# Algomorph/LevelSetFusion-Python

Hardware: AMD Instinct MI355X
Metric: voxel-warp-updates/sec (higher is better)
Workload: dtype f32

## Files before the change

### levelsetfusion-python_amd/csrc/lsf_slavcheva.hip

```cpp
#include "lsf_device.h"

using namespace lsf;

#include "lsf_slavcheva_terms.h"

using namespace lsf::slav;

namespace {


template <int D, int SMOOTH, bool LEVELSET, int DATA, int ENERGY>
__device__ inline void voxel_gradient(const float* __restrict__ live, const float* __restrict__ canonical,
                                      const float* __restrict__ warp_prev, const Grid& g, const Params& p, int x,
                                      int y, int z, int i, float (&gv)[3], double (&en)[3]) {
    gv[0] = gv[1] = gv[2] = 0.0f;
    const float l = live[i], cn = canonical[i];
    if (fabsf(l) == 1.0f && fabsf(cn) == 1.0f) return;
    const bool interior = x > 0 && x < g.nx - 1 && y > 0 && y < g.ny - 1 && (D == 2 || (z > 0 && z < g.nz - 1));
    if (g.fast_ok && __all(interior)) {
        const NbhFast<D> n(live, warp_prev, g, x, y, z);
        band_voxel_gradient<D, SMOOTH, LEVELSET, DATA, ENERGY>(n, p, l, cn, gv, en);
    } else {
        const Nbh<D> n(live, warp_prev, g, x, y, z);
        band_voxel_gradient<D, SMOOTH, LEVELSET, DATA, ENERGY>(n, p, l, cn, gv, en);
// ... 295 lines not shown
}

__global__ __launch_bounds__(1024) void band_scan_kernel(int* __restrict__ sums_base, unsigned n, unsigned stride,
                                                         unsigned arrays, long long* totals,
                                                         const int* __restrict__ opposite) {
    if (blockIdx.x >= arrays) {
        reduce_opposite(opposite, n, totals);
        return;
    }
    __shared__ int wave_total[1024 / kWave];
    int* __restrict__ sums = sums_base + (size_t)blockIdx.x * stride;
    const unsigned t = threadIdx.x, lane = t & (kWave - 1), wave = t / kWave;
    int carry = 0;
    for (unsigned base = 0; base < n; base += 4096u) {
        const unsigned i = base + 4u * t;
        int v[4];
#pragma unroll
        for (int k = 0; k < 4; ++k) v[k] = i + k < n ? sums[i + k] : 0;
        const int mine = v[0] + v[1] + v[2] + v[3];
        int inclusive = mine;
#pragma unroll
        for (int d = 1; d < kWave; d <<= 1) {
            const int up = __shfl_up(inclusive, d, kWave);
            if ((int)lane >= d) inclusive += up;
        }
        if (lane == kWave - 1) wave_total[wave] = inclusive;
        __syncthreads();
        int before = 0, tile = 0;
#pragma unroll
        for (int w = 0; w < 1024 / kWave; ++w) {
            const int x = wave_total[w];
            before += w < (int)wave ? x : 0;
            tile += x;
        }
        int run = carry + before + inclusive - mine;
#pragma unroll
        for (int k = 0; k < 4; ++k) {
            if (i + k < n) sums[i + k] = run;
            run += v[k];
        }
        carry += tile;
        __syncthreads();
    }
    if (t == 0) totals[blockIdx.x] = carry;
}

constexpr unsigned kScanTile = 4096u;

__global__ __launch_bounds__(1024) void band_tile_totals_kernel(const int* __restrict__ sums_base, unsigned n,
                                                                unsigned stride, const int* __restrict__ opposite,
                                                                int* __restrict__ tile_out, unsigned tiles) {
    __shared__ int s_sum[1024 / kWave], s_first[1024 / kWave];
    const unsigned tile = blockIdx.x, a = blockIdx.y, t = threadIdx.x;
    const unsigned i = tile * kScanTile + 4u * t;
    int sum = 0, first = 0x7fffffff;
    if (a < 2u) {
        const int* __restrict__ sums = sums_base + (size_t)a * stride;
#pragma unroll
        for (unsigned k = 0; k < 4u; ++k) sum += i + k < n ? sums[i + k] : 0;
    } else {
#pragma unroll
        for (unsigned k = 0; k < 4u; ++k)
            if (i + k < n) {
                sum += opposite[2 * (i + k)];
                first = min(first, opposite[2 * (i + k) + 1]);
            }
    }
    for (int d = kWave / 2; d > 0; d >>= 1) {
        sum += __shfl_down(sum, d, kWave);
        first = min(first, __shfl_down(first, d, kWave));
    }
    if ((t & (kWave - 1)) == 0) {
        s_sum[t / kWave] = sum;
        s_first[t / kWave] = first;
    }
    __syncthreads();
    if (t == 0) {
        for (int k = 1; k < 1024 / kWave; ++k) {
            sum += s_sum[k];
            first = min(first, s_first[k]);
        }
        tile_out[(size_t)a * tiles + tile] = sum;
        if (a == 2u) tile_out[(size_t)3 * tiles + tile] = first;
    }
}

__global__ __launch_bounds__(1024) void band_scan_tiles_kernel(int* __restrict__ sums_base, unsigned n, unsigned stride,
                                                               const int* __restrict__ tile_out, unsigned tiles,
                                                               long long* __restrict__ totals, int zero_fifth) {
    const unsigned tile = blockIdx.x, a = blockIdx.y, t = threadIdx.x, lane = t & (kWave - 1), wave = t / kWave;
    if (a == 2u) {
        if (tile == 0u && t == 0u) {
            if (zero_fifth) totals[4] = 0;
            long long sum = 0;
            int first = 0x7fffffff;
            for (unsigned k = 0; k < tiles; ++k) {
                sum += tile_out[(size_t)2 * tiles + k];
                first = min(first, tile_out[(size_t)3 * tiles + k]);
            }
            totals[2] = sum;
            totals[3] = first == 0x7fffffff ? -1 : first;
        }
        return;
    }
    __shared__ int wave_total[1024 / kWave];
    int* __restrict__ sums = sums_base + (size_t)a * stride;
    int carry = 0;
    for (unsigned k = 0; k < tile; ++k) carry += tile_out[(size_t)a * tiles + k];
    const unsigned i = tile * kScanTile + 4u * t;
    int v[4];
#pragma unroll
    for (int k = 0; k < 4; ++k) v[k] = i + k < n ? sums[i + k] : 0;
    const int mine = v[0] + v[1] + v[2] + v[3];
    int inclusive = mine;
#pragma unroll
    for (int d = 1; d < kWave; d <<= 1) {
        const int up = __shfl_up(inclusive, d, kWave);
        if ((int)lane >= d) inclusive += up;
    }
    if (lane == kWave - 1) wave_total[wave] = inclusive;
    __syncthreads();
    int before = 0, whole = 0;
#pragma unroll
    for (int w = 0; w < 1024 / kWave; ++w) {
        const int x = wave_total[w];
        before += w < (int)wave ? x : 0;
        whole += x;
    }
    int run = carry + before + inclusive - mine;
#pragma unroll
    for (int k = 0; k < 4; ++k) {
        if (i + k < n) sums[i + k] = run;
        run += v[k];
    }
    if (tile == tiles - 1u && t == 0u) totals[a] = (long long)carry + whole;
}

typedef float vf4 __attribute__((ext_vector_type(4)));

__global__ __launch_bounds__(kBlock) void state_prepare_kernel(const float* __restrict__ live,
                                                               const float* __restrict__ canonical,
                                                               vf4* __restrict__ a, vf4* __restrict__ b, unsigned n,
                                                               Grid g, int dims, int* __restrict__ sums_interior,
                                                               int* __restrict__ sums_boundary,
                                                               unsigned long long* __restrict__ masks,
                                                               int* __restrict__ opposite, int* __restrict__ nonempty) {
    __shared__ int part[4][16];
    const int t = threadIdx.x, wave = t / kWave, lane = t % kWave;
#pragma unroll
    for (int j = 0; j < 4; ++j) {
        const unsigned v = blockIdx.x * kBandChunk + j * kBlock + t;
        bool in_band = false, interior = false, opposed = false;
        if (v < n) {
            const float l = live[v], cn = canonical[v];
            in_band = !(fabsf(l) == 1.0f && fabsf(cn) == 1.0f);
            opposed = !in_band && l != cn;
            vf4 o;
            o.x = l; o.y = 0.0f; o.z = 0.0f; o.w = 0.0f;
            if (a) a[v] = o;
            if (b) b[v] = o;
            const unsigned zy = fast_div(v, g.div_nx);
            const int x = (int)(v - zy * (unsigned)g.nx);
            const int z = (int)fast_div(zy, g.div_ny);
            const int y = (int)zy - z * g.ny;
            interior = x > 0 && x < g.nx - 1 && y > 0 && y < g.ny - 1 && (dims == 2 || (z > 0 && z < g.nz - 1));
        }
        const unsigned long long mi = __ballot(in_band && interior), mb = __ballot(in_band && !interior);
        const unsigned long long mo = __ballot(opposed);
        if (lane == 0) {
            part[0][j * 4 + wave] = __popcll(mi);
            part[1][j * 4 + wave] = __popcll(mb);
            part[2][j * 4 + wave] = __popcll(mo);
            part[3][j * 4 + wave] = mo ? (int)(blockIdx.x * kBandChunk + j * kBlock + wave * kWave) + __ffsll((long long)mo) - 1
                                       : 0x7fffffff;
            masks[((size_t)blockIdx.x * 16 + j * 4 + wave) * 2 + 0] = mi;
            masks[((size_t)blockIdx.x * 16 + j * 4 + wave) * 2 + 1] = mb;
        }
    }
    __syncthreads();
    if (t < 2) {
        int sum = 0;
        for (int k = 0; k < 16; ++k) sum += part[t][k];
        (t == 0 ? sums_interior : sums_boundary)[blockIdx.x] = sum;
    } else if (t == 2) {
        int sum = 0, first = 0x7fffffff;
        for (int k = 0; k < 16; ++k) {
            sum += part[2][k];
            first = min(first, part[3][k]);
        }
        opposite[2 * blockIdx.x] = sum;
        opposite[2 * blockIdx.x + 1] = first;
    } else if (t == 3) {
        int any = 0;
        for (int k = 0; k < 16; ++k) any |= part[0][k] | part[1][k];
        nonempty[blockIdx.x] = any != 0;
    }
}

constexpr int kPrepareChunksPerBlock = 4;
__device__ inline unsigned long long row16_or(unsigned nibble, int lane) {
    const int pos = lane & 15;
    unsigned lo = pos < 8 ? nibble << (4 * pos) : 0u, hi = pos < 8 ? 0u : nibble << (4 * (pos - 8));
#pragma unroll
    for (int d = 1; d < 16; d <<= 1) {
        lo |= (unsigned)__shfl_xor((int)lo, d, kWave);
        hi |= (unsigned)__shfl_xor((int)hi, d, kWave);
    }
    return ((unsigned long long)hi << 32) | lo;
}

__global__ __launch_bounds__(kBlock) void state_prepare4_kernel(const vf4* __restrict__ live4,
                                                                const vf4* __restrict__ canonical4,
                                                                vf4* __restrict__ a, vf4* __restrict__ b, unsigned n,
                                                                unsigned chunks, Grid g, int dims,
                                                                int* __restrict__ sums_interior,
                                                                int* __restrict__ sums_boundary,
                                                                unsigned long long* __restrict__ masks,
                                                                int* __restrict__ opposite, int* __restrict__ nonempty) {
    __shared__ int part[kPrepareChunksPerBlock][4][16];
    const int t = threadIdx.x, wave = t / kWave, lane = t % kWave;
    const unsigned chunk0 = blockIdx.x * kPrepareChunksPerBlock;
    vf4 l[kPrepareChunksPerBlock], c[kPrepareChunksPerBlock];
#pragma unroll
    for (int k = 0; k < kPrepareChunksPerBlock; ++k) {
        const unsigned v = (chunk0 + k) * kBandChunk + 4u * t;
        const vf4 one = {1.0f, 1.0f, 1.0f, 1.0f};
        l[k] = v < n ? live4[v / 4] : one;
        c[k] = v < n ? canonical4[v / 4] : one;
    }
#pragma unroll
    for (int k = 0; k < kPrepareChunksPerBlock; ++k) {
        const unsigned chunk = chunk0 + k, v = chunk * kBandChunk + 4u * t;
        unsigned ni = 0u, nb = 0u, no = 0u;
        if (v < n) {
            const unsigned zy = fast_div(v, g.div_nx);
            const int x0 = (int)(v - zy * (unsigned)g.nx);
            const int z = (int)fast_div(zy, g.div_ny);
            const int y = (int)zy - z * g.ny;
            const bool row_inside = y > 0 && y < g.ny - 1 && (dims == 2 || (z > 0 && z < g.nz - 1));
            const float lv[4] = {l[k].x, l[k].y, l[k].z, l[k].w}, cv[4] = {c[k].x, c[k].y, c[k].z, c[k].w};
#pragma unroll
            for (int j = 0; j < 4; ++j) {
                const bool in_band = !(fabsf(lv[j]) == 1.0f && fabsf(cv[j]) == 1.0f);
                const bool interior = row_inside && x0 + j > 0 && x0 + j < g.nx - 1;
                ni |= (in_band && interior ? 1u : 0u) << j;
                nb |= (in_band && !interior ? 1u : 0u) << j;
                no |= (!in_band && lv[j] != cv[j] ? 1u : 0u) << j;
                vf4 o;
                o.x = lv[j]; o.y = 0.0f; o.z = 0.0f; o.w = 0.0f;
                if (a) a[v + j] = o;
                if (b) b[v + j] = o;
            }
        }
        const unsigned long long mi = row16_or(ni, lane), mb = row16_or(nb, lane), mo = row16_or(no, lane);
        if ((lane & 15) == 0 && chunk < chunks) {
            const int word = wave * 4 + lane / 16;
            part[k][0][word] = __popcll(mi);
            part[k][1][word] = __popcll(mb);
            part[k][2][word] = __popcll(mo);
            part[k][3][word] = mo ? (int)(chunk * kBandChunk + word * kWave) + __ffsll((long long)mo) - 1 : 0x7fffffff;
            masks[((size_t)chunk * 16 + word) * 2 + 0] = mi;
            masks[((size_t)chunk * 16 + word) * 2 + 1] = mb;
        }
    }
    __syncthreads();
    if (t < 4 * kPrepareChunksPerBlock) {
        const int k = t / 4, what = t % 4;
        const unsigned chunk = chunk0 + k;
        if (chunk < chunks) {
            if (what < 2) {
                int sum = 0;
                for (int w = 0; w < 16; ++w) sum += part[k][what][w];
                (what == 0 ? sums_interior : sums_boundary)[chunk] = sum;
            } else if (what == 2) {
                int sum = 0, first = 0x7fffffff;
                for (int w = 0; w < 16; ++w) {
                    sum += part[k][2][w];
                    first = min(first, part[k][3][w]);
                }
                opposite[2 * chunk] = sum;
                opposite[2 * chunk + 1] = first;
            } else {
                int any = 0;
                for (int w = 0; w < 16; ++w) any |= part[k][0][w] | part[k][1][w];
                nonempty[chunk] = any != 0;
            }
        }
    }
}

__device__ inline bool chunk_is_needed(unsigned c, unsigned chunks, long long row, long long slice, int dims, int reach,
                                       const int* __restrict__ nonempty) {
    const int lane = threadIdx.x % kWave;
    const long long c0 = (long long)c * kBandChunk;
    const int span = 2 * reach + 1, zs = dims == 3 ? span : 1;
    bool hit = false;
    for (int k = lane; k < zs * span; k += kWave) {
        const int dy = k % span - reach, dz = dims == 3 ? k / span - reach : 0;
        const long long lo = c0 + dz * slice + dy * row - reach, hi = c0 + (long long)kBandChunk - 1 + dz * slice + dy * row + reach;
        long long first = lo >= 0 ? lo / kBandChunk : -((-lo + kBandChunk - 1) / kBandChunk);
        long long last = hi >= 0 ? hi / kBandChunk : -((-hi + kBandChunk - 1) / kBandChunk);
        first = first < 0 ? 0 : first;
        last = last >= (long long)chunks ? (long long)chunks - 1 : last;
        for (long long cand = first; cand <= last; ++cand) hit |= nonempty[cand] != 0;
    }
    return __any(hit);
}

constexpr int kPackChunks = 1;
static_assert(kPackChunks <= kBlock / kWave, "a wave per chunk of the block forms the verdicts");
__global__ __launch_bounds__(kBlock) void state_pack_needed_kernel(const float* __restrict__ live, vf4* __restrict__ a,
                                                                   vf4* __restrict__ b, unsigned n, unsigned chunks,
                                                                   int* __restrict__ needed, int want, int reach,
                                                                   long long row, long long slice, int dims,
                                                                   const int* __restrict__ nonempty) {
    const int t = threadIdx.x;
    __shared__ int s_verdict[kPackChunks];
    if (reach > 0) {
        const int k = t / kWave;
        const unsigned c = blockIdx.x * kPackChunks + k;
        if (k < kPackChunks && c < chunks) {
            const int any = chunk_is_needed(c, chunks, row, slice, dims, reach, nonempty) ? 1 : 0;
            if (t % kWave == 0) {
                needed[c] = any;
                s_verdict[k] = any;
            }
        }
        __syncthreads();
    }
    int verdict[kPackChunks];
#pragma unroll
    for (int k = 0; k < kPackChunks; ++k) {
        const unsigned c = blockIdx.x * kPackChunks + k;
        verdict[k] = c < chunks ? (reach > 0 ? s_verdict[k] : needed[c]) : -1;
    }
#pragma unroll
    for (int k = 0; k < kPackChunks; ++k) {
        if (verdict[k] != want) continue;
        const unsigned c = blockIdx.x * kPackChunks + k;
#pragma unroll
        for (int j = 0; j < 4; ++j) {
            const unsigned v = c * kBandChunk + j * kBlock + t;
            if (v < n) {
                vf4 o;
                o.x = live[v]; o.y = 0.0f; o.z = 0.0f; o.w = 0.0f;
                if (a) a[v] = o;
                if (b) b[v] = o;
            }
        }
    }
}



__global__ __launch_bounds__(kBlock) void band_fill_from_masks_kernel(const unsigned long long* __restrict__ masks,
                                                                      const int* __restrict__ block_sums, int which,
                                                                      int* __restrict__ list, unsigned chunks) {
    const int lane = threadIdx.x % kWave;
    const unsigned chunk = blockIdx.x * (kBlock / kWave) + threadIdx.x / kWave;
    if (chunk >= chunks) return;
    const unsigned long long mine = lane < 16 ? masks[((size_t)chunk * 16 + lane) * 2 + which] : 0ull;
    if (__ballot(mine != 0ull) == 0ull) return;
    int at = block_sums[chunk];
#pragma unroll
    for (int w = 0; w < 16; ++w) {
        const unsigned lo = (unsigned)__shfl((int)(unsigned)mine, w, kWave);
        const unsigned hi = (unsigned)__shfl((int)(unsigned)(mine >> 32), w, kWave);
        const unsigned long long m = ((unsigned long long)hi << 32) | lo;
        if ((m >> lane) & 1ull)
            list[at + __popcll(m & ((1ull << lane) - 1ull))] = (int)(chunk * kBandChunk + w * kWave + lane);
        at += __popcll(m);
    }
}

}

static inline bool band_subset_ok(int32_t subset) {
    return subset == LSF_BAND_ALL || subset == LSF_BAND_INTERIOR || subset == LSF_BAND_BOUNDARY;
}

extern "C" int lsf_slavcheva_gradient(const float* live, const float* canonical, const float* warp_prev_planar,
                                      float* g_out_planar, const lsf_grid* grid, const lsf_slavcheva_params* params,
                                      const lsf_gate* gate, lsf_iteration_record* record, const int32_t* band_list,
                                      int64_t band_count, void* stream) {
    if (int e = check_grid(grid)) return e;
    if (!live || !canonical || !warp_prev_planar || !params || !record || !g_out_planar ||
        g_out_planar == warp_prev_planar || (band_list && (band_count < 0 || band_count > 0x7fffffffll)))
        return LSF_ERR_BAD_ARGUMENT;
    Grid g = make_grid(grid);
    Tiling t = make_tiling(g);
    if (t.total == 0) return 0;
    LaunchArgs a{band_list ? band_list_blocks((unsigned)band_count) : launch_blocks(t.total), as_stream(stream), live,
                 canonical, warp_prev_planar, g_out_planar, g, make_params(params), gate_or_open(gate), record, band_list,
                 (unsigned)band_count};
    if (grid->dims == 2) pick_terms<2>(params, a);
    else pick_terms<3>(params, a);
    return launch_status();
}

extern "C" int lsf_slavcheva_update_rewarp(const float* live, const float* canonical, float* g_planar,
                                           float* warp_out_planar, float* live_out, const lsf_grid* grid,
                                           const lsf_slavcheva_params* params, const lsf_gate* gate,
                                           lsf_iteration_record* record, const int32_t* band_list, int64_t band_count,
                                           void* stream) {
    (void)canonical;
    if (int e = check_grid(grid)) return e;
    if (!live || !g_planar || !warp_out_planar || !live_out || live_out == live || !params || !record ||
        (band_list && (band_count < 0 || band_count > 0x7fffffffll)))
        return LSF_ERR_BAD_ARGUMENT;
    Grid g = make_grid(grid);
    Tiling t = make_tiling(g);
    if (t.total == 0) return 0;
    Params p = make_params(params);
    lsf_gate gt = gate_or_open(gate);
    const unsigned blocks = band_list ? band_list_blocks((unsigned)band_count) : launch_blocks(t.total);
    if (grid->dims == 2)
        hipLaunchKernelGGL(slavcheva_update_rewarp_kernel<2>, dim3(blocks), dim3(kBlock), 0, as_stream(stream), live,
                           g_planar, warp_out_planar, live_out, g, p, gt, record, band_list, (unsigned)band_count);
    else
        hipLaunchKernelGGL(slavcheva_update_rewarp_kernel<3>, dim3(blocks), dim3(kBlock), 0, as_stream(stream), live,
                           g_planar, warp_out_planar, live_out, g, p, gt, record, band_list, (unsigned)band_count);
    return launch_status();
}

template <int D, int NT>
static void launch_filter_update(bool fma, unsigned blocks, hipStream_t s, const float* in, const float* mask,
                                 const float* live, float* g_out, float* warp_out, float* live_out, const Grid& g,
                                 const Params& p, const double* taps_host, int axis, const lsf_gate& gt,
                                 lsf_iteration_record* record, const int* list, unsigned count) {
    TapsN<NT> taps;
    for (int j = 0; j < NT; ++j) taps.k[j] = taps_host[j];
    if (fma)
        hipLaunchKernelGGL((slavcheva_filter_update_rewarp_kernel<D, NT, true>), dim3(blocks), dim3(kBlock), 0, s, in, mask,
                           live, g_out, warp_out, live_out, g, p, taps, axis, gt, record, list, count);
    else
        hipLaunchKernelGGL((slavcheva_filter_update_rewarp_kernel<D, NT, false>), dim3(blocks), dim3(kBlock), 0, s, in, mask,
                           live, g_out, warp_out, live_out, g, p, taps, axis, gt, record, list, count);
}

extern "C" int lsf_slavcheva_filter_update_rewarp(const float* in_planar, const float* zero_mask_source,
                                                  const float* live, float* g_out_planar, float* warp_out_planar,
                                                  float* live_out, const lsf_grid* grid,
                                                  const lsf_slavcheva_params* params, int32_t axis,
                                                  const double* taps_host, int32_t n_taps, const lsf_gate* gate,
                                                  lsf_iteration_record* record, const int32_t* band_list,
                                                  int64_t band_count, void* stream) {
    if (int e = check_grid(grid)) return e;
    if (!in_planar || !zero_mask_source || !live || !g_out_planar || !warp_out_planar || !live_out ||
        live_out == live || g_out_planar == in_planar || !params || !record || !taps_host || !band_list ||
        band_count < 0 || band_count > 0x7fffffffll || axis < 0 || axis >= grid->dims)
        return LSF_ERR_BAD_ARGUMENT;
    if (n_taps != 3 && n_taps != 5 && n_taps != 7 && n_taps != 9) return LSF_ERR_KERNEL_TOO_LONG;
    Grid g = make_grid(grid);
    if (g.z_end == g.z_begin) return 0;
    const Params p = make_params(params);
    const lsf_gate gt = gate_or_open(gate);
    const unsigned blocks = band_list_blocks((unsigned)band_count);
    hipStream_t s = as_stream(stream);
    bool fma = true;
    for (int j = 0; j < n_taps; ++j) fma = fma && (double)(float)taps_host[j] == taps_host[j];
    const int* list = band_list;
    const unsigned count = (unsigned)band_count;
#define LSF_FUR(D, NT) launch_filter_update<D, NT>(fma, blocks, s, in_planar, zero_mask_source, live, g_out_planar, \
                                                 warp_out_planar, live_out, g, p, taps_host, axis, gt, record, list, count)
    if (grid->dims == 2) {
        switch (n_taps) { case 3: LSF_FUR(2, 3); break; case 5: LSF_FUR(2, 5); break; case 7: LSF_FUR(2, 7); break; default: LSF_FUR(2, 9); break; }
    } else {
        switch (n_taps) { case 3: LSF_FUR(3, 3); break; case 5: LSF_FUR(3, 5); break; case 7: LSF_FUR(3, 7); break; default: LSF_FUR(3, 9); break; }
    }
#undef LSF_FUR
    return launch_status();
}

static inline bool band_range(const lsf_grid* grid, unsigned& first, unsigned& n, unsigned& chunks) {
    const long long slice = (long long)grid->ny * grid->nx;
    first = (unsigned)(slice * grid->z_begin);
    n = (unsigned)(slice * (grid->z_end - grid->z_begin));
    chunks = (n + kBandChunk - 1) / kBandChunk;
    return n > 0;
}

extern "C" int64_t lsf_band_scratch_elements(const lsf_grid* grid) {
    if (check_grid(grid)) return 0;
    unsigned first, n, chunks;
    band_range(grid, first, n, chunks);
    return (int64_t)chunks + 1;
}

extern "C" int lsf_band_count(const float* live, const float* canonical, const lsf_grid* grid, int32_t subset,
                              int32_t* scratch, int64_t* count_out, void* stream) {
    if (int e = check_grid(grid)) return e;
    if (!live || !canonical || !scratch || !count_out || !band_subset_ok(subset)) return LSF_ERR_BAD_ARGUMENT;
    unsigned first, n, chunks;
    band_range(grid, first, n, chunks);
    hipStream_t s = as_stream(stream);
    if (chunks > 0)
        hipLaunchKernelGGL(band_list_kernel<false>, dim3(chunks), dim3(kBlock), 0, s, live, canonical, first, n,
                           make_grid(grid), grid->dims, subset, scratch, (int*)nullptr);
    hipLaunchKernelGGL(band_scan_kernel, dim3(1), dim3(1024), 0, s, scratch, chunks, 0u, 1u, (long long*)count_out,
                       (const int*)nullptr);
    return launch_status();
}

static inline unsigned long long* prepare_masks(int32_t* scratch, unsigned chunks) {
    return reinterpret_cast<unsigned long long*>(scratch + 2 * (size_t)(chunks + 1) + (2 * (chunks + 1)) % 2);
}

static inline int* prepare_opposite(int32_t* scratch, unsigned chunks) {
    return reinterpret_cast<int*>(prepare_masks(scratch, chunks) + (size_t)chunks * 32);
}

static inline int* prepare_nonempty(int32_t* scratch, unsigned chunks) { return prepare_opposite(scratch, chunks) + 2 * (size_t)chunks; }
static inline int* prepare_needed(int32_t* scratch, unsigned chunks) { return prepare_nonempty(scratch, chunks) + chunks; }
static inline unsigned prepare_scan_tiles(unsigned chunks) { return (chunks + kScanTile - 1u) / kScanTile; }
static inline int* prepare_tile_totals(int32_t* scratch, unsigned chunks) { return prepare_needed(scratch, chunks) + chunks; }

extern "C" int64_t lsf_state_prepare_scratch_elements(const lsf_grid* grid) {
    if (check_grid(grid, true)) return 0;
    unsigned first, n, chunks;
    band_range(grid, first, n, chunks);
    return 2 * (int64_t)(chunks + 1) + 64 * (int64_t)chunks + 2 + 2 * (int64_t)chunks + 2 * (int64_t)chunks +
           4 * ((int64_t)prepare_scan_tiles(chunks) + 1);
}

extern "C" int lsf_band_list_fill_prepared(const lsf_grid* grid, int32_t subset, const int32_t* scratch, int32_t* list,
                                           void* stream) {
    if (int e = check_grid(grid, true)) return e;
    if (!scratch || !list || (subset != LSF_BAND_INTERIOR && subset != LSF_BAND_BOUNDARY) || grid->z_begin != 0 ||
        grid->z_end != grid->nz)
        return LSF_ERR_BAD_ARGUMENT;
    unsigned first, n, chunks;
    if (!band_range(grid, first, n, chunks)) return 0;
    const int which = subset == LSF_BAND_INTERIOR ? 0 : 1;
    hipLaunchKernelGGL(band_fill_from_masks_kernel, dim3((chunks + kBlock / kWave - 1) / (kBlock / kWave)), dim3(kBlock),
                       0, as_stream(stream), prepare_masks(const_cast<int32_t*>(scratch), chunks),
                       scratch + which * (size_t)(chunks + 1), which, list, chunks);
    return launch_status();
}

namespace {
constexpr int kBoxGroup = kBlock;

__device__ inline unsigned long long box_mask_of(const unsigned long long* __restrict__ masks, unsigned box, int nbx,
                                                 int nby, int nx, int ny, bool all) {
    const int bx = (int)(box % (unsigned)nbx), by = (int)((box / (unsigned)nbx) % (unsigned)nby);
    const int bz = (int)(box / ((unsigned)nbx * (unsigned)nby));
    unsigned long long m = 0ull;
#pragma unroll
    for (int k = 0; k < 4; ++k)
#pragma unroll
        for (int j = 0; j < 4; ++j) {
            const unsigned v = (unsigned)(((4 * bz + k) * ny + 4 * by + j) * nx + 4 * bx);
            const unsigned long long word = masks[2 * (size_t)(v >> 6)] | (all ? masks[2 * (size_t)(v >> 6) + 1] : 0ull);
            m |= ((word >> (v & 63u)) & 0xFull) << (4 * (k * 4 + j));
        }
    return m;
}

template <bool FILL>
__global__ __launch_bounds__(kBlock) void band_boxes_kernel(const unsigned long long* __restrict__ masks, unsigned n_boxes,
                                                            int nbx, int nby, int nx, int ny, bool all,
                                                            int* __restrict__ group_sums, lsf_band_box* __restrict__ boxes) {
    __shared__ int wave_count[kBlock / kWave];
    const unsigned box = blockIdx.x * kBoxGroup + threadIdx.x;
    const int lane = threadIdx.x % kWave, wave = threadIdx.x / kWave;
    const unsigned long long m = box < n_boxes ? box_mask_of(masks, box, nbx, nby, nx, ny, all) : 0ull;
    const unsigned long long any = __ballot(m != 0ull);
    if (lane == 0) wave_count[wave] = __popcll(any);
    __syncthreads();
    if (!FILL) {
        if (threadIdx.x == 0) {
            int sum = 0;
            for (int k = 0; k < kBlock / kWave; ++k) sum += wave_count[k];
            group_sums[blockIdx.x] = sum;
        }
        return;
    }
    if (m == 0ull) return;
    int at = group_sums[blockIdx.x];
    for (int k = 0; k < wave; ++k) at += wave_count[k];
    at += __popcll(any & ((1ull << lane) - 1ull));
    const int bx = (int)(box % (unsigned)nbx), by = (int)((box / (unsigned)nbx) % (unsigned)nby);
    const int bz = (int)(box / ((unsigned)nbx * (unsigned)nby));
    lsf_band_box b;
    b.origin = ((4 * bz) * ny + 4 * by) * nx + 4 * bx;
    b.reserved = 0;
    b.mask = m;
    boxes[at] = b;
}

inline bool boxes_ok(const lsf_grid* g) {
    return g->dims == 3 && g->nx % 4 == 0 && g->ny % 4 == 0 && g->nz % 4 == 0 && g->z_begin == 0 && g->z_end == g->nz &&
           (long long)g->nx * g->ny * g->nz <= 0x0fffffffll;
}
}

extern "C" int64_t lsf_band_boxes_scratch_elements(const lsf_grid* grid) {
    if (check_grid(grid) || !boxes_ok(grid)) return 0;
    const long long n_boxes = (long long)grid->nx * grid->ny * grid->nz / 64;
    return (n_boxes + kBoxGroup - 1) / kBoxGroup + 1;
}

extern "C" int lsf_band_boxes_count(const lsf_grid* grid, int32_t subset, const int32_t* prepare_scratch,
                                    int32_t* box_scratch, int64_t* count_out, void* stream) {
    if (int e = check_grid(grid)) return e;
    if (!boxes_ok(grid)) return LSF_ERR_BAD_DIMS;
    if (!prepare_scratch || !box_scratch || !count_out || (subset != LSF_BAND_INTERIOR && subset != LSF_BAND_ALL))
        return LSF_ERR_BAD_ARGUMENT;
    unsigned first, n, chunks;
    band_range(grid, first, n, chunks);
    const unsigned n_boxes = n / 64, groups = (n_boxes + kBoxGroup - 1) / kBoxGroup;
    hipStream_t s = as_stream(stream);
    hipLaunchKernelGGL(band_boxes_kernel<false>, dim3(groups), dim3(kBlock), 0, s,
                       prepare_masks(const_cast<int32_t*>(prepare_scratch), chunks), n_boxes, grid->nx / 4, grid->ny / 4,
                       grid->nx, grid->ny, subset == LSF_BAND_ALL, box_scratch, (lsf_band_box*)nullptr);
    hipLaunchKernelGGL(band_scan_kernel, dim3(1), dim3(1024), 0, s, box_scratch, groups, 0u, 1u, (long long*)count_out,
                       (const int*)nullptr);
    return launch_status();
}

extern "C" int lsf_band_boxes_fill(const lsf_grid* grid, int32_t subset, const int32_t* prepare_scratch,
                                   const int32_t* box_scratch, lsf_band_box* boxes, void* stream) {
    if (int e = check_grid(grid)) return e;
    if (!boxes_ok(grid)) return LSF_ERR_BAD_DIMS;
    if (!prepare_scratch || !box_scratch || !boxes || (subset != LSF_BAND_INTERIOR && subset != LSF_BAND_ALL))
        return LSF_ERR_BAD_ARGUMENT;
    unsigned first, n, chunks;
    band_range(grid, first, n, chunks);
    const unsigned n_boxes = n / 64, groups = (n_boxes + kBoxGroup - 1) / kBoxGroup;
    hipLaunchKernelGGL(band_boxes_kernel<true>, dim3(groups), dim3(kBlock), 0, as_stream(stream),
                       prepare_masks(const_cast<int32_t*>(prepare_scratch), chunks), n_boxes, grid->nx / 4, grid->ny / 4,
                       grid->nx, grid->ny, subset == LSF_BAND_ALL, const_cast<int32_t*>(box_scratch), boxes);
    return launch_status();
}

extern "C" int lsf_state_prepare(const float* live, const float* canonical, float* state_a, float* state_b,
                                 const lsf_grid* grid, int32_t* scratch, int64_t* counts_out, void* stream) {
    return state_prepare_launch(live, canonical, state_a, state_b, grid, scratch, counts_out, false, stream);
}

int lsf::state_prepare_launch(const float* live, const float* canonical, float* state_a, float* state_b, const lsf_grid* grid,
                              int32_t* scratch, int64_t* counts_out, bool zero_fifth, void* stream) {
    if (int e = check_grid(grid, true)) return e;
    if (!live || !canonical || (!state_a && state_b) || !scratch || !counts_out) return LSF_ERR_BAD_ARGUMENT;
    if (grid->z_begin != 0 || grid->z_end != grid->nz) return LSF_ERR_BAD_ARGUMENT;
    unsigned first, n, chunks;
    band_range(grid, first, n, chunks);
    hipStream_t s = as_stream(stream);
    int* sums_interior = scratch;
    int* sums_boundary = scratch + (chunks + 1);
    const bool wide = grid->nx % 4 == 0 && ((uintptr_t)live | (uintptr_t)canonical) % 16 == 0;
    if (wide)
        hipLaunchKernelGGL(state_prepare4_kernel, dim3((chunks + kPrepareChunksPerBlock - 1) / kPrepareChunksPerBlock),
                           dim3(kBlock), 0, s, reinterpret_cast<const vf4*>(live), reinterpret_cast<const vf4*>(canonical),
                           reinterpret_cast<vf4*>(state_a), reinterpret_cast<vf4*>(state_b), n, chunks, make_grid(grid),
                           grid->dims, sums_interior, sums_boundary, prepare_masks(scratch, chunks),
                           prepare_opposite(scratch, chunks), prepare_nonempty(scratch, chunks));
    else
        hipLaunchKernelGGL(state_prepare_kernel, dim3(chunks), dim3(kBlock), 0, s, live, canonical,
                           reinterpret_cast<vf4*>(state_a), reinterpret_cast<vf4*>(state_b), n, make_grid(grid), grid->dims,
                           sums_interior, sums_boundary, prepare_masks(scratch, chunks), prepare_opposite(scratch, chunks),
                           prepare_nonempty(scratch, chunks));
    const unsigned tiles = prepare_scan_tiles(chunks) > 0u ? prepare_scan_tiles(chunks) : 1u;
    hipLaunchKernelGGL(band_tile_totals_kernel, dim3(tiles, 3), dim3(1024), 0, s, scratch, chunks, chunks + 1,
                       (const int*)prepare_opposite(scratch, chunks), prepare_tile_totals(scratch, chunks), tiles);
    hipLaunchKernelGGL(band_scan_tiles_kernel, dim3(tiles, 3), dim3(1024), 0, s, scratch, chunks, chunks + 1,
                       (const int*)prepare_tile_totals(scratch, chunks), tiles, (long long*)counts_out, zero_fifth ? 1 : 0);
    return launch_status();
}

extern "C" int lsf_state_pack_needed(const float* live, float* state_a, float* state_b, const lsf_grid* grid,
                                     int32_t* scratch, int32_t reach, int32_t invert, void* stream) {
    if (int e = check_grid(grid, true)) return e;
    if (!live || (!state_a && !state_b) || !scratch || reach < 1 || reach > 8) return LSF_ERR_BAD_ARGUMENT;
    if (grid->z_begin != 0 || grid->z_end != grid->nz) return LSF_ERR_BAD_ARGUMENT;
    unsigned first, n, chunks;
    band_range(grid, first, n, chunks);
    hipLaunchKernelGGL(state_pack_needed_kernel, dim3((chunks + kPackChunks - 1) / kPackChunks), dim3(kBlock), 0,
                       as_stream(stream), live, reinterpret_cast<vf4*>(state_a), reinterpret_cast<vf4*>(state_b), n, chunks,
                       prepare_needed(scratch, chunks), invert ? 0 : 1, invert ? 0 : (int)reach, (long long)grid->nx,
                       (long long)grid->nx * grid->ny, grid->dims, (const int*)prepare_nonempty(scratch, chunks));
    return launch_status();
}

extern "C" int lsf_band_list_fill(const float* live, const float* canonical, const lsf_grid* grid, int32_t subset,
                                  const int32_t* scratch, int32_t* list, void* stream) {
    if (int e = check_grid(grid)) return e;
    if (!live || !canonical || !scratch || !list || !band_subset_ok(subset)) return LSF_ERR_BAD_ARGUMENT;
    unsigned first, n, chunks;
    if (!band_range(grid, first, n, chunks)) return 0;
    hipLaunchKernelGGL(band_list_kernel<true>, dim3(chunks), dim3(kBlock), 0, as_stream(stream), live, canonical, first, n,
                       make_grid(grid), grid->dims, subset, const_cast<int32_t*>(scratch), list);
    return launch_status();
}
```

### levelsetfusion-python_amd/device.py

```python
import ctypes

import numpy as np
import torch

from . import _lib
from ._lib import Gate, Grid, HierParams, SlavchevaParams, check, lib
from .device_core import *
from .device_core import _PINNED, _gate_ref, _ptr, _record_ptr
from .device_fields import *
from .device_terms import term_gradient

def hier_iteration(packed, canonical, warp, g_prev, g_out, grid, params, gate, records, index):
    n = n_voxels(grid)
    n_packed = params.packed_nz * grid.ny * grid.nx if params.packed_nz > 0 else n
    check(lib.lsf_hier_iteration(_ptr(packed, 4 * n_packed, "packed live"), _ptr(canonical, n, "canonical"),
                                 _ptr(warp, n * grid.dims, "warp"),
                                 _ptr(g_prev, n * grid.dims, "g_prev", allow_none=True),
                                 _ptr(g_out, n * grid.dims, "g_out", allow_none=True), ctypes.byref(grid),
                                 ctypes.byref(params), _gate_ref(gate), _record_ptr(records, index), stream_ptr()),
          "lsf_hier_iteration")


def hier_update(g, warp, grid, rate, gate, records, index):
    n = n_voxels(grid) * grid.dims
    check(lib.lsf_hier_update(_ptr(g, n, "g"), _ptr(warp, n, "warp", allow_none=True), ctypes.byref(grid), float(rate),
                              _gate_ref(gate), _record_ptr(records, index), stream_ptr()), "lsf_hier_update")


class BandList:

    def __init__(self, indices, count, subset=_lib.BAND_ALL):
        self.indices, self.count, self.subset = indices, int(count), int(subset)
        self.pointer = ctypes.c_void_p(indices.data_ptr() if indices is not None else 0)

    @classmethod
    def none(cls):
        return cls(None, 0)


def buffer_addressing_ok(grid, bytes_per_voxel=16):
    if bytes_per_voxel != 16:
        return bytes_per_voxel * n_voxels(grid) < 0xffffffff
    return n_voxels(grid) < 0x7fffffff and 16 * (2 * grid.nx * grid.ny + 2 * grid.nx + 3) < 0x7fffffff


def band_lists(live, canonical, grid=None, split=True, bytes_per_voxel=16):
    grid = grid or make_grid(live.shape)
    n = n_voxels(grid)
    subsets = (_lib.BAND_INTERIOR, _lib.BAND_BOUNDARY) if split and buffer_addressing_ok(grid, bytes_per_voxel) \
        else (_lib.BAND_ALL,)
    n_scratch = int(lib.lsf_band_scratch_elements(ctypes.byref(grid)))
    scratch = torch.empty((len(subsets), n_scratch), dtype=torch.int32, device=live.device)
    totals = torch.zeros(len(subsets), dtype=torch.int64, device=live.device)
    p_live, p_canon = _ptr(live, n, "live"), _ptr(canonical, n, "canonical")
    for k, subset in enumerate(subsets):
        check(lib.lsf_band_count(p_live, p_canon, ctypes.byref(grid), subset, ctypes.c_void_p(scratch[k].data_ptr()),
                                 ctypes.c_void_p(totals[k:].data_ptr()), stream_ptr()), "lsf_band_count")
    counts = [int(c) for c in totals.cpu()]
    lists = []
    for k, (subset, count) in enumerate(zip(subsets, counts)):
        if count == 0 and not (k == len(subsets) - 1 and not lists):
            continue
        indices = torch.empty(max(count, 1), dtype=torch.int32, device=live.device)
        if count:
            check(lib.lsf_band_list_fill(p_live, p_canon, ctypes.byref(grid), subset,
                                         ctypes.c_void_p(scratch[k].data_ptr()), ctypes.c_void_p(indices.data_ptr()),
                                         stream_ptr()), "lsf_band_list_fill")
        lists.append(BandList(indices, count, subset))
    return lists


def band_list(live, canonical, grid=None, subset=_lib.BAND_ALL):
    grid = grid or make_grid(live.shape)
    n = n_voxels(grid)
    scratch = torch.empty(int(lib.lsf_band_scratch_elements(ctypes.byref(grid))), dtype=torch.int32,
                          device=live.device)
    total = torch.zeros(1, dtype=torch.int64, device=live.device)
    p_live, p_canon = _ptr(live, n, "live"), _ptr(canonical, n, "canonical")
    check(lib.lsf_band_count(p_live, p_canon, ctypes.byref(grid), int(subset), ctypes.c_void_p(scratch.data_ptr()),
                             ctypes.c_void_p(total.data_ptr()), stream_ptr()), "lsf_band_count")
    count = int(total.item())
    indices = torch.empty(max(count, 1), dtype=torch.int32, device=live.device)
    if count:
        check(lib.lsf_band_list_fill(p_live, p_canon, ctypes.byref(grid), int(subset),
                                     ctypes.c_void_p(scratch.data_ptr()), ctypes.c_void_p(indices.data_ptr()),
                                     stream_ptr()), "lsf_band_list_fill")
    return BandList(indices, count, subset)


def slavcheva_gradient(live, canonical, warp_prev, g_out, grid, params, gate, records, index, band=None):
    n = n_voxels(grid)
    nd = n * grid.dims
    check(lib.lsf_slavcheva_gradient(_ptr(live, n, "live"), _ptr(canonical, n, "canonical"),
                                     _ptr(warp_prev, nd, "warp_prev"), _ptr(g_out, nd, "g_out"), ctypes.byref(grid),
                                     ctypes.byref(params), _gate_ref(gate), _record_ptr(records, index),
                                     band.pointer if band is not None else ctypes.c_void_p(0),
                                     band.count if band is not None else 0, stream_ptr()),
          "lsf_slavcheva_gradient")


class StatePrepare:

    CHUNK = 1024
    SPLIT_MAX_VOXELS = 1 << 24

    def __init__(self, live, canonical, grid=None, cut_chunks=None, sparse_reach=0):
        self.grid = grid = grid or make_grid(live.shape)
        n = n_voxels(grid)
        self.states = [torch.empty(tuple(live.shape) + (4,), dtype=torch.float32, device=live.device) for _ in range(2)]
        n_scratch = int(lib.lsf_state_prepare_scratch_elements(ctypes.byref(grid)))
        self._scratch = torch.empty(n_scratch, dtype=torch.int32, device=live.device)
        totals = torch.empty(4, dtype=torch.int64, device=live.device)
        self.sparse_reach = int(sparse_reach)
        split = n <= self.SPLIT_MAX_VOXELS
        none = ctypes.c_void_p(0)
        check(lib.lsf_state_prepare(_ptr(live, n, "live"), _ptr(canonical, n, "canonical"),
                                    none if self.sparse_reach else _ptr(self.states[0], 4 * n, "state"),
                                    none if split or self.sparse_reach else _ptr(self.states[1], 4 * n, "state"),
                                    ctypes.byref(grid), ctypes.c_void_p(self._scratch.data_ptr()),
                                    ctypes.c_void_p(totals.data_ptr()), stream_ptr()), "lsf_state_prepare")
        self._totals_host = pinned_scratch("prepare totals", 4, torch.int64)
        self._totals_host.copy_(totals, non_blocking=True)
        self._cuts_host = self._cut_chunks = None
        if cut_chunks is not None and cut_chunks.numel():
            chunks = (n + self.CHUNK - 1) // self.CHUNK
            prefix = self._scratch[:2 * (chunks + 1)].view(2, chunks + 1)
            cuts = torch.index_select(prefix, 1, cut_chunks)
            self._cuts_host = pinned_scratch("prepare cuts", cuts.numel(), torch.int32)
            self._cuts_host.copy_(cuts.view(-1), non_blocking=True)
        self._copied = torch.cuda.Event()
        self._copied.record()
        if self.sparse_reach:
            check(lib.lsf_state_pack_needed(_ptr(live, n, "live"), _ptr(self.states[0], 4 * n, "state"),
                                            _ptr(self.states[1], 4 * n, "state"), ctypes.byref(full_range(grid)),
                                            ctypes.c_void_p(self._scratch.data_ptr()), self.sparse_reach, 0,
                                            stream_ptr()), "lsf_state_pack_needed")
        elif split:
            check(lib.lsf_state_pack(_ptr(live, n, "live"), ctypes.c_void_p(0), _ptr(self.states[1], 4 * n, "state"),
                                     ctypes.c_void_p(0), ctypes.byref(full_range(grid)), stream_ptr()), "lsf_state_pack")

    def complete(self, state, live):
        if not self.sparse_reach:
            return state
        n = n_voxels(self.grid)
        check(lib.lsf_state_pack_needed(_ptr(live, n, "live"), _ptr(state, 4 * n, "state"), ctypes.c_void_p(0),
                                        ctypes.byref(full_range(self.grid)), ctypes.c_void_p(self._scratch.data_ptr()),
                                        self.sparse_reach, 1, stream_ptr()), "lsf_state_pack_needed")
        return state

    def needed_fraction(self):
        n = n_voxels(self.grid)
        chunks = (n + self.CHUNK - 1) // self.CHUNK
        at = 2 * (chunks + 1) + 64 * chunks + 2 * chunks + chunks
        return float(self._scratch[at:at + chunks].ne(0).float().mean().item())

    def collect(self):
        self._copied.synchronize()
        counts = self._totals_host.tolist()
        p_scratch = ctypes.c_void_p(self._scratch.data_ptr())
        lists = []
        for k, (subset, count) in enumerate(zip((_lib.BAND_INTERIOR, _lib.BAND_BOUNDARY), counts[:2])):
            if count == 0 and not (k == 1 and not lists):
                continue
            indices = torch.empty(max(count, 1), dtype=torch.int32, device=self._scratch.device)
            if count:
                check(lib.lsf_band_list_fill_prepared(ctypes.byref(self.grid), subset, p_scratch,
                                                      ctypes.c_void_p(indices.data_ptr()), stream_ptr()),
                      "lsf_band_list_fill_prepared")
            lists.append(BandList(indices, count, subset))
        self.cuts = None
        if self._cuts_host is not None:
            flat = self._cuts_host.tolist()
            per = len(flat) // 2
            self.cuts = {subset: flat[k * per:(k + 1) * per]
                         for k, subset in enumerate((_lib.BAND_INTERIOR, _lib.BAND_BOUNDARY))}
            self.cut_totals = {_lib.BAND_INTERIOR: counts[0], _lib.BAND_BOUNDARY: counts[1]}
        return lists, (counts[2], counts[3])


def state_prepare(live, canonical, grid=None):
    prepared = StatePrepare(live, canonical, grid)
    lists, unlisted = prepared.collect()
    return prepared.states, lists, unlisted


def state_pack(live, warp_planar=None, grid=None, copies=2):
    grid = grid or make_grid(live.shape)
    n = n_voxels(grid)
    states = [torch.empty(tuple(live.shape) + (4,), dtype=torch.float32, device=live.device) for _ in range(copies)]
    check(lib.lsf_state_pack(_ptr(live, n, "live"), _ptr(warp_planar, n * grid.dims, "warp", allow_none=True),
                             _ptr(states[0], 4 * n, "state"),
                             _ptr(states[1], 4 * n, "state") if copies > 1 else ctypes.c_void_p(0),
                             ctypes.byref(full_range(grid)), stream_ptr()), "lsf_state_pack")
    return states


def state_unpack(state, grid, live_out=None, warp_planar_out=None, warp_interleaved_out=None):
    n = n_voxels(grid)
    check(lib.lsf_state_unpack(_ptr(state, 4 * n, "state"), _ptr(live_out, n, "live_out", allow_none=True),
                               _ptr(warp_planar_out, n * grid.dims, "warp_planar_out", allow_none=True),
                               _ptr(warp_interleaved_out, n * grid.dims, "warp_interleaved_out", allow_none=True),
                               ctypes.byref(full_range(grid)), stream_ptr()), "lsf_state_unpack")


def state_finalize(state, canonical, grid, live_out=None, warp_planar_out=None, warp_interleaved_out=None,
                   lower_threshold=0.0, statistics=False):
    n = n_voxels(grid)
    stats = scratch = None
    if statistics:
        stats = torch.empty(16, dtype=torch.float64, device=state.device)
        scratch = torch.empty(int(lib.lsf_state_finalize_scratch_elements(ctypes.byref(grid))), dtype=torch.float64,
                              device=state.device)
    check(lib.lsf_state_finalize(_ptr(state, 4 * n, "state"), _ptr(canonical, n, "canonical", allow_none=not statistics),
                                 _ptr(live_out, n, "live_out", allow_none=True),
                                 _ptr(warp_planar_out, n * grid.dims, "warp_planar_out", allow_none=True),
                                 _ptr(warp_interleaved_out, n * grid.dims, "warp_interleaved_out", allow_none=True),
                                 ctypes.byref(grid), float(lower_threshold),
                                 _ptr(stats, 16, "statistics", dtype=torch.float64, allow_none=True),
                                 _ptr(scratch, scratch.numel() if scratch is not None else 0, "scratch",
                                      dtype=torch.float64, allow_none=True), stream_ptr()), "lsf_state_finalize")
    return stats


def planar_finalize(live, warp_planar, canonical, grid, live_out=None, warp_interleaved_out=None, lower_threshold=0.0,
                    statistics=False):
    n = n_voxels(grid)
    stats = scratch = None
    if statistics:
        stats = torch.empty(16, dtype=torch.float64, device=live.device)
        scratch = torch.empty(int(lib.lsf_state_finalize_scratch_elements(ctypes.byref(grid))), dtype=torch.float64,
                              device=live.device)
    check(lib.lsf_planar_finalize(_ptr(live, n, "live"), _ptr(warp_planar, n * grid.dims, "warp"),
                                  _ptr(canonical, n, "canonical", allow_none=not statistics),
                                  _ptr(live_out, n, "live_out", allow_none=True),
                                  _ptr(warp_interleaved_out, n * grid.dims, "warp_interleaved_out", allow_none=True),
                                  ctypes.byref(grid), float(lower_threshold),
                                  _ptr(stats, 16, "statistics", dtype=torch.float64, allow_none=True),
                                  _ptr(scratch, scratch.numel() if scratch is not None else 0, "scratch",
                                       dtype=torch.float64, allow_none=True), stream_ptr()), "lsf_planar_finalize")
    return stats


def state_finalize_listed(state, canonical, grid, bands, unlisted, live_out=None, warp_interleaved_out=None,
                          lower_threshold=0.0, statistics=False, skip_flag=None, guard=None):
    n = n_voxels(grid)
    bands = [b for b in bands if b.count]
    stats = scratch = None
    if statistics:
        stats = torch.empty(16, dtype=torch.float64, device=state.device)
        scratch = torch.empty(int(lib.lsf_state_finalize_scratch_elements(ctypes.byref(grid))) * max(len(bands), 1),
                              dtype=torch.float64, device=state.device)
    pointers = (ctypes.c_void_p * 2)(*[b.pointer for b in bands])
    counts = (ctypes.c_int64 * 2)(*[b.count for b in bands])
    check(lib.lsf_state_finalize_listed(_ptr(state, 4 * n, "state"),
                                        _ptr(canonical, n, "canonical", allow_none=not statistics),
                                        _ptr(live_out, n, "live_out", allow_none=True),
                                        _ptr(warp_interleaved_out, n * grid.dims, "warp_interleaved_out",
                                             allow_none=True),
                                        ctypes.byref(grid), pointers, counts, len(bands), int(unlisted[0]),
                                        int(unlisted[1]), float(lower_threshold),
                                        _ptr(stats, 16, "statistics", dtype=torch.float64, allow_none=True),
                                        _ptr(scratch, scratch.numel() if scratch is not None else 0, "scratch",
                                             dtype=torch.float64, allow_none=True),
                                        ctypes.c_void_p(skip_flag or 0),
                                        ctypes.c_void_p(guard[0].data_ptr() if guard is not None else 0),
                                        int(guard[1]) if guard is not None else 0,
                                        float(guard[2]) if guard is not None else 0.0, stream_ptr()),
          "lsf_state_finalize_listed")
    return stats


BOX_EDGE = 4


def boxes_ok(grid):
    return (grid.dims == 3 and grid.nx % BOX_EDGE == 0 and grid.ny % BOX_EDGE == 0 and grid.nz % BOX_EDGE == 0
            and n_voxels(grid) <= 0x0fffffff)


def band_boxes(prepared, subset=_lib.BAND_INTERIOR):
    grid = full_range(prepared.grid)
    scratch = torch.empty(int(lib.lsf_band_boxes_scratch_elements(ctypes.byref(grid))), dtype=torch.int32,
                          device=prepared._scratch.device)
    count = torch.zeros(1, dtype=torch.int64, device=scratch.device)
    p_prepare = ctypes.c_void_p(prepared._scratch.data_ptr())
    check(lib.lsf_band_boxes_count(ctypes.byref(grid), subset, p_prepare, ctypes.c_void_p(scratch.data_ptr()),
                                   ctypes.c_void_p(count.data_ptr()), stream_ptr()), "lsf_band_boxes_count")
    n = int(count.item())
    boxes = torch.empty((max(n, 1), 2), dtype=torch.int64, device=scratch.device)
    if n:
        check(lib.lsf_band_boxes_fill(ctypes.byref(grid), subset, p_prepare, ctypes.c_void_p(scratch.data_ptr()),
                                      ctypes.c_void_p(boxes.data_ptr()), stream_ptr()), "lsf_band_boxes_fill")
    return boxes, n


def band_boxes_canonical(canonical, grid, boxes, n_boxes):
    out = torch.empty(max(n_boxes, 1) * BOX_EDGE ** 3, dtype=torch.float32, device=canonical.device)
    check(lib.lsf_band_boxes_canonical(_ptr(canonical, n_voxels(grid), "canonical"), ctypes.byref(grid),
                                       ctypes.c_void_p(boxes.data_ptr()), int(n_boxes), ctypes.c_void_p(out.data_ptr()),
                                       stream_ptr()), "lsf_band_boxes_canonical")
    return out


def slavcheva_state_iteration_boxes(state_in, canonical_boxed, state_out, grid, params, gate, records, index, boxes, n_boxes):
    n = n_voxels(grid)
    check(lib.lsf_slavcheva_state_iteration_boxes(_ptr(state_in, 4 * n, "state_in"),
                                                  _ptr(canonical_boxed, n_boxes * BOX_EDGE ** 3, "canonical_boxed"),
                                                  _ptr(state_out, 4 * n, "state_out"), ctypes.byref(grid),
                                                  ctypes.byref(params), _gate_ref(gate), _record_ptr(records, index),
                                                  ctypes.c_void_p(boxes.data_ptr()), int(n_boxes), stream_ptr()),
          "lsf_slavcheva_state_iteration_boxes")


def full_range(grid):
    g = Grid.from_buffer_copy(grid)
    g.z_begin, g.z_end = 0, g.nz
    return g


def slavcheva_state_iteration(state_in, canonical, state_out, grid, params, gate, records, index, band=None):
    n = n_voxels(grid)
    check(lib.lsf_slavcheva_state_iteration(_ptr(state_in, 4 * n, "state_in"), _ptr(canonical, n, "canonical"),
                                            _ptr(state_out, 4 * n, "state_out"), ctypes.byref(grid),
                                            ctypes.byref(params), _gate_ref(gate), _record_ptr(records, index),
                                            band.pointer if band is not None else ctypes.c_void_p(0),
                                            band.count if band is not None else 0,
                                            band.subset if band is not None else 0, stream_ptr()),
          "lsf_slavcheva_state_iteration")


def cumulative_warp_compose(state, psi_in, psi_out, grid, gate=None, band=None):
    n = n_voxels(grid)
    check(lib.lsf_cumulative_warp_compose(_ptr(state, 4 * n, "state"), _ptr(psi_in, 4 * n, "psi_in"),
                                          _ptr(psi_out, 4 * n, "psi_out"), ctypes.byref(grid), _gate_ref(gate),
                                          band.pointer if band is not None else ctypes.c_void_p(0),
                                          band.count if band is not None else 0, stream_ptr()),
          "lsf_cumulative_warp_compose")


def slavcheva_update_rewarp(live, canonical, g, warp_out, live_out, grid, params, gate, records, index, band=None):
    n = n_voxels(grid)
    nd = n * grid.dims
    check(lib.lsf_slavcheva_update_rewarp(_ptr(live, n, "live"), _ptr(canonical, n, "canonical"), _ptr(g, nd, "g"),
                                          _ptr(warp_out, nd, "warp_out"), _ptr(live_out, n, "live_out"),
                                          ctypes.byref(grid), ctypes.byref(params), _gate_ref(gate),
                                          _record_ptr(records, index),
                                          band.pointer if band is not None else ctypes.c_void_p(0),
                                          band.count if band is not None else 0, stream_ptr()),
          "lsf_slavcheva_update_rewarp")


def slavcheva_filter_update_rewarp(src, mask_source, live, g_out, warp_out, live_out, grid, params, axis, taps, gate,
                                   records, index, band):
    taps = np.ascontiguousarray(np.asarray(taps, dtype=np.float64))
    n = n_voxels(grid)
    nd = n * grid.dims
    check(lib.lsf_slavcheva_filter_update_rewarp(_ptr(src, nd, "filter src"), _ptr(mask_source, nd, "zero mask"),
                                                 _ptr(live, n, "live"), _ptr(g_out, nd, "g_out"),
                                                 _ptr(warp_out, nd, "warp_out"), _ptr(live_out, n, "live_out"),
                                                 ctypes.byref(grid), ctypes.byref(params), int(axis),
                                                 taps.ctypes.data_as(ctypes.POINTER(ctypes.c_double)), taps.size,
                                                 _gate_ref(gate), _record_ptr(records, index), band.pointer, band.count,
                                                 stream_ptr()), "lsf_slavcheva_filter_update_rewarp")


class IterationLauncher:

    def __init__(self, grid, records, gate_mode, gate_a, gate_b=0.0):
        self.grid = grid
        self.grid_ref = ctypes.byref(grid)
        self.records = records
        n = records.shape[0]
        base = records.data_ptr()
        self.record_ptrs = [ctypes.c_void_p(base + i * _lib.RECORD_BYTES) for i in range(n)]
        self.gates = [Gate(base + i * _lib.RECORD_BYTES, int(gate_mode), float(gate_a), float(gate_b))
                      for i in range(n)]
        self.gate_refs = [ctypes.byref(g) for g in self.gates]
        self._keep = []

    def pointer(self, t, numel, name, allow_none=False):
        p = _ptr(t, numel, name, allow_none=allow_none)
        self._keep.append(t)
        return p

    def gate_ref(self, prev_index):
        return None if prev_index is None or prev_index < 0 else self.gate_refs[prev_index]


def warp_statistics(warp_planar, canonical, live, lower_threshold, grid=None):
    grid = grid or make_grid(live.shape)
    n = n_voxels(grid)
    out = torch.empty(8, dtype=torch.float64, device=live.device)
    check(lib.lsf_warp_statistics(_ptr(warp_planar, n * grid.dims, "warp"), _ptr(canonical, n, "canonical"),
                                  _ptr(live, n, "live"), ctypes.byref(grid), float(lower_threshold),
                                  _ptr(out, 8, "out8", dtype=torch.float64), stream_ptr()), "lsf_warp_statistics")
    return out


def tsdf_difference_statistics(canonical, live, grid=None):
    grid = grid or make_grid(live.shape)
    n = n_voxels(grid)
    out = torch.empty(8, dtype=torch.float64, device=live.device)
    check(lib.lsf_tsdf_difference_statistics(_ptr(canonical, n, "canonical"), _ptr(live, n, "live"),
                                             ctypes.byref(grid), _ptr(out, 8, "out8", dtype=torch.float64),
                                             stream_ptr()), "lsf_tsdf_difference_statistics")
    return out
```

Baseline: 531.7 billion.

## Pack sparse state at 32-voxel group granularity using band bitmasks

The needed-chunk pack kernel now refines each needed 1024-voxel chunk into 32 groups of 32 voxels. Each group's verdict comes from checking the band bitmasks over its neighbourhood reach, and only voxels in needed groups are loaded and written. The per-chunk nonempty scan is also unrolled to three fixed loads instead of a variable loop. The aim is to cut state writes and live reads on large grids, paid for by extra bitmask reads, a block sync per chunk, and an env-controlled threshold for small grids.

```diff
diff --git a/levelsetfusion-python_amd/csrc/lsf_slavcheva.hip b/levelsetfusion-python_amd/csrc/lsf_slavcheva.hip
--- a/levelsetfusion-python_amd/csrc/lsf_slavcheva.hip
+++ b/levelsetfusion-python_amd/csrc/lsf_slavcheva.hip
@@ -621,56 +621,99 @@
         long long last = hi >= 0 ? hi / kBandChunk : -((-hi + kBandChunk - 1) / kBandChunk);
         first = first < 0 ? 0 : first;
         last = last >= (long long)chunks ? (long long)chunks - 1 : last;
-        for (long long cand = first; cand <= last; ++cand) hit |= nonempty[cand] != 0;
+        int flag[3];
+#pragma unroll
+        for (int j = 0; j < 3; ++j) flag[j] = first + j <= last ? nonempty[first + j] : 0;
+        hit |= (flag[0] | flag[1] | flag[2]) != 0;
     }
     return __any(hit);
 }
 
-constexpr int kPackChunks = 1;
-static_assert(kPackChunks <= kBlock / kWave, "a wave per chunk of the block forms the verdicts");
+constexpr int kPackGroup = 32;
+constexpr int kPackGroups = (int)kBandChunk / kPackGroup;
+static_assert(kPackGroups == 32 && kWave == 2 * kPackGroups && kBlock % kPackGroups == 0,
+              "a chunk's verdicts fill the int kept per chunk; two half waves per ballot");
+__device__ inline unsigned group_verdicts_of_wave(unsigned c, unsigned chunks, long long row, long long slice, int dims,
+                                                  int reach, const unsigned long long* __restrict__ masks) {
+    const int span = 2 * reach + 1, offsets = span * (dims == 3 ? span : 1);
+    const long long bits = (long long)chunks * kBandChunk;
+    const long long g0 = (long long)c * kBandChunk + (threadIdx.x % kPackGroups) * kPackGroup;
+    constexpr int kStep = kBlock / kPackGroups, kBatch = 4;
+    bool hit = false;
+    for (int k0 = threadIdx.x / kPackGroups; k0 < offsets; k0 += kBatch * kStep) {
+        unsigned long long first[kBatch], second[kBatch], upto[kBatch];
+        bool one[kBatch];
+#pragma unroll
+        for (int u = 0; u < kBatch; ++u) {
+            const int k = k0 + u * kStep;
+            const int dy = k % span - reach, dz = dims == 3 ? k / span - reach : 0;
+            long long lo = g0 + dz * slice + dy * row - reach, hi = g0 + kPackGroup - 1 + dz * slice + dy * row + reach;
+            lo = lo < 0 ? 0 : lo;
+            hi = hi >= bits ? bits - 1 : hi;
+            const bool inside = k < offsets && lo <= hi;
+            const long long w0 = inside ? lo >> 6 : 0, w1 = inside ? hi >> 6 : 0;
+            first[u] = (masks[2 * w0] | masks[2 * w0 + 1]) & (inside ? ~0ull << (lo & 63) : 0ull);
+            second[u] = masks[2 * w1] | masks[2 * w1 + 1];
+            upto[u] = ~0ull >> (63 - (hi & 63));
+            one[u] = w0 == w1;
+        }
+#pragma unroll
+        for (int u = 0; u < kBatch; ++u)
+            hit |= (one[u] ? first[u] & upto[u] : first[u] | (second[u] & upto[u])) != 0ull;
+    }
+    const unsigned long long both = __ballot(hit);
+    return (unsigned)both | (unsigned)(both >> 32);
+}
+
 __global__ __launch_bounds__(kBlock) void state_pack_needed_kernel(const float* __restrict__ live, vf4* __restrict__ a,
                                                                    vf4* __restrict__ b, unsigned n, unsigned chunks,
                                                                    int* __restrict__ needed, int want, int reach,
                                                                    long long row, long long slice, int dims,
-                                                                   const int* __restrict__ nonempty) {
+                                                                   const int* __restrict__ nonempty,
+                                                                   const unsigned long long* __restrict__ masks,
+                                                                   int groups) {
     const int t = threadIdx.x;
-    __shared__ int s_verdict[kPackChunks];
+    const unsigned c = blockIdx.x;
+    __shared__ unsigned s_share[kBlock / kWave];
+    unsigned mask;
     if (reach > 0) {
-        const int k = t / kWave;
-        const unsigned c = blockIdx.x * kPackChunks + k;
-        if (k < kPackChunks && c < chunks) {
-            const int any = chunk_is_needed(c, chunks, row, slice, dims, reach, nonempty) ? 1 : 0;
-            if (t % kWave == 0) {
-                needed[c] = any;
-                s_verdict[k] = any;
-            }
-        }
-        __syncthreads();
-    }
-    int verdict[kPackChunks];
-#pragma unroll
-    for (int k = 0; k < kPackChunks; ++k) {
-        const unsigned c = blockIdx.x * kPackChunks + k;
-        verdict[k] = c < chunks ? (reach > 0 ? s_verdict[k] : needed[c]) : -1;
-    }
-#pragma unroll
-    for (int k = 0; k < kPackChunks; ++k) {
-        if (verdict[k] != want) continue;
-        const unsigned c = blockIdx.x * kPackChunks + k;
-#pragma unroll
-        for (int j = 0; j < 4; ++j) {
-            const unsigned v = c * kBandChunk + j * kBlock + t;
-            if (v < n) {
-                vf4 o;
-                o.x = live[v]; o.y = 0.0f; o.z = 0.0f; o.w = 0.0f;
-                if (a) a[v] = o;
-                if (b) b[v] = o;
-            }
-        }
-    }
-}
-
-
+        if (!chunk_is_needed(c, chunks, row, slice, dims, reach, nonempty)) {
+            if (t == 0) needed[c] = 0;
+            return;
+        }
+        if (!groups) {
+            if (t == 0) needed[c] = 1;
+            mask = ~0u;
+        } else {
+            const unsigned share = group_verdicts_of_wave(c, chunks, row, slice, dims, reach, masks);
+            if (t % kWave == 0) s_share[t / kWave] = share;
+            __syncthreads();
+            mask = 0u;
+#pragma unroll
+            for (int w = 0; w < kBlock / kWave; ++w) mask |= s_share[w];
+            if (t == 0) needed[c] = (int)mask;
+        }
+    } else {
+        mask = groups ? (unsigned)needed[c] : needed[c] != 0 ? ~0u : 0u;
+    }
+    if (want == 0) mask = ~mask;
+    float l[4];
+#pragma unroll
+    for (int j = 0; j < 4; ++j) {
+        const unsigned at = j * kBlock + t, v = c * kBandChunk + at;
+        l[j] = ((mask >> (at / kPackGroup)) & 1u) != 0u && v < n ? live[v] : 0.0f;
+    }
+#pragma unroll
+    for (int j = 0; j < 4; ++j) {
+        const unsigned at = j * kBlock + t, v = c * kBandChunk + at;
+        if (((mask >> (at / kPackGroup)) & 1u) != 0u && v < n) {
+            vf4 o;
+            o.x = l[j]; o.y = 0.0f; o.z = 0.0f; o.w = 0.0f;
+            if (a) a[v] = o;
+            if (b) b[v] = o;
+        }
+    }
+}
 
 __global__ __launch_bounds__(kBlock) void band_fill_from_masks_kernel(const unsigned long long* __restrict__ masks,
                                                                       const int* __restrict__ block_sums, int which,
@@ -988,6 +1031,14 @@
     return launch_status();
 }
 
+static long long pack_group_min_voxels() {
+    const char* text = std::getenv("LSF_SPARSE_MIN_VOXELS");
+    if (!text || !*text) return 1ll << 21;
+    char* end = nullptr;
+    const long long value = std::strtoll(text, &end, 10);
+    return end && *end == 0 && value >= 0 ? value : 1ll << 21;
+}
+
 extern "C" int lsf_state_pack_needed(const float* live, float* state_a, float* state_b, const lsf_grid* grid,
                                      int32_t* scratch, int32_t reach, int32_t invert, void* stream) {
     if (int e = check_grid(grid, true)) return e;
@@ -995,10 +1046,12 @@
     if (grid->z_begin != 0 || grid->z_end != grid->nz) return LSF_ERR_BAD_ARGUMENT;
     unsigned first, n, chunks;
     band_range(grid, first, n, chunks);
-    hipLaunchKernelGGL(state_pack_needed_kernel, dim3((chunks + kPackChunks - 1) / kPackChunks), dim3(kBlock), 0,
-                       as_stream(stream), live, reinterpret_cast<vf4*>(state_a), reinterpret_cast<vf4*>(state_b), n, chunks,
+    hipLaunchKernelGGL(state_pack_needed_kernel, dim3(chunks), dim3(kBlock), 0, as_stream(stream), live,
+                       reinterpret_cast<vf4*>(state_a), reinterpret_cast<vf4*>(state_b), n, chunks,
                        prepare_needed(scratch, chunks), invert ? 0 : 1, invert ? 0 : (int)reach, (long long)grid->nx,
-                       (long long)grid->nx * grid->ny, grid->dims, (const int*)prepare_nonempty(scratch, chunks));
+                       (long long)grid->nx * grid->ny, grid->dims, (const int*)prepare_nonempty(scratch, chunks),
+                       (const unsigned long long*)prepare_masks(scratch, chunks),
+                       (long long)n >= pack_group_min_voxels() ? 1 : 0);
     return launch_status();
 }
 
diff --git a/levelsetfusion-python_amd/device.py b/levelsetfusion-python_amd/device.py
--- a/levelsetfusion-python_amd/device.py
+++ b/levelsetfusion-python_amd/device.py
@@ -1,4 +1,5 @@
 import ctypes
+import os
 
 import numpy as np
 import torch
@@ -102,16 +103,19 @@
 class StatePrepare:
 
     CHUNK = 1024
+    GROUP = 32
     SPLIT_MAX_VOXELS = 1 << 24
 
-    def __init__(self, live, canonical, grid=None, cut_chunks=None, sparse_reach=0):
+    def __init__(self, live, canonical, grid=None, cut_chunks=None, sparse_reach=0, states=None):
         self.grid = grid = grid or make_grid(live.shape)
         n = n_voxels(grid)
-        self.states = [torch.empty(tuple(live.shape) + (4,), dtype=torch.float32, device=live.device) for _ in range(2)]
+        self.states = list(states) if states is not None else [
+            torch.empty(tuple(live.shape) + (4,), dtype=torch.float32, device=live.device) for _ in range(2)]
         n_scratch = int(lib.lsf_state_prepare_scratch_elements(ctypes.byref(grid)))
         self._scratch = torch.empty(n_scratch, dtype=torch.int32, device=live.device)
         totals = torch.empty(4, dtype=torch.int64, device=live.device)
         self.sparse_reach = int(sparse_reach)
+        self._groups = n >= self.group_min_voxels()
         split = n <= self.SPLIT_MAX_VOXELS
         none = ctypes.c_void_p(0)
         check(lib.lsf_state_prepare(_ptr(live, n, "live"), _ptr(canonical, n, "canonical"),
@@ -148,11 +152,27 @@
                                         self.sparse_reach, 1, stream_ptr()), "lsf_state_pack_needed")
         return state
 
-    def needed_fraction(self):
+    @staticmethod
+    def group_min_voxels():
+        text = os.environ.get("LSF_SPARSE_MIN_VOXELS", "")
+        return int(text) if text.isdigit() else 1 << 21
+
+    def _needed_words(self):
         n = n_voxels(self.grid)
         chunks = (n + self.CHUNK - 1) // self.CHUNK
         at = 2 * (chunks + 1) + 64 * chunks + 2 * chunks + chunks
-        return float(self._scratch[at:at + chunks].ne(0).float().mean().item())
+        return self._scratch[at:at + chunks]
+
+    def needed_masks(self):
+        words = self._needed_words()
+        return words if self._groups else -words.ne(0).to(torch.int32)
+
+    def needed_fraction(self):
+        return float(self._needed_words().ne(0).float().mean().item())
+
+    def written_fraction(self):
+        masks = self.needed_masks().cpu().numpy().view(np.uint32)
+        return float(np.unpackbits(masks.view(np.uint8)).mean())
 
     def collect(self):
         self._copied.synchronize()
```

Result: faster. 541.6 billion, median of 6 (+1.9%).
